# karknu/ouroboros-consensus

Hardware: AMD Instinct MI355X
Metric: Praos headers validated/sec (VRF+KES+OCert+leader) (higher is better)
Workload: dtype u32 (GF(2^255-19) radix-2^32 limbs; Fixed E34 bignum); 1 GPU; configs[4]: mainnet-shaped epoch replay, the first 432k blocks of a first-leader-wins Praos chain per GPU, 3000-pool stake distribution, single eta0, 1% corrupted; items_per_gpu=432000, items_total=432000, pools=3000, active_slot_coeff=1/20, signed_body=canonical HeaderBody CBOR, parallelism=shard-by-slot-range x1

## Files before the change

### ouroboros-consensus_amd/csrc/api_internal.hpp

```cpp
#pragma once
#include "praos_hip.h"
#include "launch.hpp"
#include "host_util.hpp"
#include "replay_internal.hpp"
#include "chunk_scan.hpp"
#include "sched.hpp"

static constexpr size_t NT = 256;
static constexpr size_t NIELS_BYTES = 3 * 32;
static constexpr size_t BTAB_N = 128;
static constexpr size_t BCOMB_TABLES = 32;
static constexpr size_t C16_TABLES = 16, C16_ENTRIES = 32768;
static constexpr size_t CACHED_BYTES = 4 * 32;
static constexpr size_t LT_ED_B = 8 * CACHED_BYTES, LT_VRF_B = 16 * CACHED_BYTES;
static constexpr size_t VRF_MID_BYTES = 28 * 16;
static constexpr uint32_t TP_SIGNED_STRIDE = 640;

#include <pthread.h>
#include <sched.h>

#include <algorithm>
#include <array>
#include <chrono>
#include <condition_variable>
#include <cstdlib>
#include <cstdio>
#include <cstring>
#include <functional>
#include <map>
// ... 385 lines not shown
```

### ouroboros-consensus_amd/csrc/k_selftest.hpp

```cpp
#pragma once
#include "kcommon.hpp"

#if PRAOS_ILP4
#define ST_LAUNCH(name) launch_selftest4_##name
#else
#define ST_LAUNCH(name) launch_selftest_##name
#endif

template <int BUILD>
__global__ void __launch_bounds__(64) k_selftest_fe_multi(int op, size_t n, const uint8_t* __restrict__ in,
                                                          uint8_t* __restrict__ out) {
  const size_t i = (size_t)blockIdx.x * blockDim.x + threadIdx.x;
  if (i >= n) return;
  fe a[4], b[4], r[4];
#pragma unroll
  for (int m = 0; m < 4; m++) {
    load_words(a[m].v, in + 256 * i + 64 * m, 8);
    load_words(b[m].v, in + 256 * i + 64 * m + 32, 8);
    fe_set(r[m], 0);
  }
  switch (op) {
    case 0: fe_mul2(r[0], a[0], b[0], r[1], a[1], b[1]); break;
    case 1: fe_sq2(r[0], a[0], r[1], a[1]); break;
    case 2: fe_mul3(r[0], a[0], b[0], r[1], a[1], b[1], r[2], a[2], b[2]); break;
// ... 178 lines not shown
    load_words(s1, sp + 32 * i, 8);
    load_words(s2, sq + 32 * i, 8);
    ge_p3 H, G;
    ge_frombytes(H, pk, false);
    load_words(pk, Qenc + 32 * i, 8);
    ge_frombytes(G, pk, false);
    fe_neg(G.X, G.X);
    fe_neg(G.T, G.T);
    ge_cached* vt = lane_tab(tabs, i, 16);
    build_cached_table(vt, H);
    build_cached_table(vt + 8, G);
    sc_recode16(w1, s1);
    sc_recode16(w2, s2);
    STRAUS<64, 64, 33, 0, false>(x, vt, w1, vt + 8, w2, nullptr, nullptr);
    ge_p1p1_to_p2(R, x);
  } else if constexpr (V == 3) {
    load_words(s1, sp + 32 * i, 8);
    load_words(s2, sb + 32 * i, 8);
    sc_recode16(w1, s1);
    sc_recode65536(w2, s2);
    straus_comb<16, false>(x, ktab + i * KT_STRIDE, w1, comb, w2);
    ge_p1p1_to_p2(R, x);
  } else if constexpr (V == 4) {
    load_words(s1, sp + 32 * i, 8);
    load_words(s2, sb + 32 * i, 8);
    sc_recode16(w1, s1);
    sc_recode65536(w2, s2);
    straus_comb<8, true>(x, ktab + i * KT_STRIDE, w1, comb, w2);
    ge_p1p1_to_p2(R, x);
  } else if constexpr (V == 6) {
// ... 2 lines not shown
    sc_recode65536(w2, s2);
    straus_pos(x, ktab + i * WT_STRIDE, s1, comb, w2);
    ge_p1p1_to_p2(R, x);
  } else {
    load_words(pk, Penc + 32 * i, 8);
    load_words(s1, sp + 32 * i, 8);
    ge_p3 P, S;
    ge_frombytes(P, pk, false);
    ge_scalarmult_var(S, s1, P);
    ge_p3_to_p2(R, S);
  }
  ge_tobytes(enc, R.X, R.Y, R.Z);
  store_words(out + 32 * i, enc, 8);
}

#if !PRAOS_ILP4
template <int BUILD>
__global__ void __launch_bounds__(64) k_selftest_int(int op, size_t n, const uint8_t* __restrict__ a,
                                                     const uint8_t* __restrict__ b, const uint8_t* __restrict__ c,
                                                     uint8_t* __restrict__ out) {
  const size_t i = (size_t)blockIdx.x * blockDim.x + threadIdx.x;
  if (i >= n) return;
  uint32_t x[8], y[8], z[8], r[8];
  load_words(x, a + 32 * i, 8);
#pragma unroll
  for (int k = 0; k < 8; k++) { y[k] = 0; z[k] = 0; r[k] = 0; }
  if (op == 1) {
    load_words(y, b + 32 * i, 8);
    load_words(z, c + 32 * i, 8);
  }
  if (op == 8) load_words(y, b + 32 * i, 8);
// ... 8 lines not shown
      uint32_t w[5];
      sc_recode64(w, x);
#pragma unroll
      for (int k = 0; k < 5; k++) r[k] = w[k];
    } break;
    case 7: fx_div_R(r, x); break;
    case 8: mp_div_small(r, x, y[0]); break;
    default: break;
  }
  store_words(out + 32 * i, r, 8);
}
#endif

void ST_LAUNCH(ge)(hipStream_t stream, int op, size_t n, const uint8_t* p, const uint8_t* q, uint8_t* out,
                   const ge_niels* gbtab) {
  hipLaunchKernelGGL(k_selftest_ge<PRAOS_ILP4>, dim3((unsigned)((n + 63) / 64)), dim3(64), 0, stream, op, n, p, q, out,
                     gbtab);
}
void ST_LAUNCH(msm)(hipStream_t stream, int variant, size_t n, const uint8_t* P, const uint8_t* Q, const uint8_t* sp,
                    const uint8_t* sq, const uint8_t* sb, const ge_niels* gbtab, const ge_niels* comb, ge_cached* tabs,
                    const ge_cached* ktab, uint8_t* out) {
  const dim3 grid((unsigned)((n + NT - 1) / NT)), block(NT);
#define ST_MSM(V)                                                                                                  \
  case V:                                                                                                          \
    hipLaunchKernelGGL((k_selftest_msm<PRAOS_ILP4, V>), grid, block, 0, stream, n, P, Q, sp, sq, sb, gbtab, comb, \
                       tabs, ktab, out);                                                                           \
    break
  switch (variant) {
    ST_MSM(0);
    ST_MSM(1);
    ST_MSM(2);
    ST_MSM(3);
    ST_MSM(4);
    ST_MSM(5);
    ST_MSM(6);
    default: break;
  }
#undef ST_MSM
}
#if !PRAOS_ILP4
void launch_selftest_fe_multi(hipStream_t stream, int op, size_t n, const uint8_t* in, uint8_t* out) {
  hipLaunchKernelGGL(k_selftest_fe_multi<0>, dim3((unsigned)((n + 63) / 64)), dim3(64), 0, stream, op, n, in, out);
}
void launch_selftest_fe(hipStream_t stream, int op, size_t n, const uint8_t* a, const uint8_t* b, uint8_t* r) {
  hipLaunchKernelGGL(k_selftest_fe<0>, dim3((unsigned)((n + 63) / 64)), dim3(64), 0, stream, op, n, a, b, r);
}
void launch_selftest_int(hipStream_t stream, int op, size_t n, const uint8_t* a, const uint8_t* b, const uint8_t* c,
                         uint8_t* out) {
  hipLaunchKernelGGL(k_selftest_int<0>, dim3((unsigned)((n + 63) / 64)), dim3(64), 0, stream, op, n, a, b, c, out);
}
#endif
```

### ouroboros-consensus_amd/csrc/k_vrf_stage.hip

```cpp
#include "k_vrf.hpp"

#ifndef LB_VRF_V
#define LB_VRF_V LB_VRF
#endif
#ifndef LB_VRF_F
#define LB_VRF_F LB_VRF
#endif
#ifndef LB_VRF_J
#define LB_VRF_J LB_VRF_F
#endif

__global__ void __launch_bounds__(NT, LB_VRF_V) k_vrf_v(size_t n, size_t i0, size_t i1, VrfIn a, uint4* __restrict__ mid) {
  const size_t i = i0 + (size_t)blockIdx.x * blockDim.x + threadIdx.x;
  if (i >= i1) return;
  if (a.wave_prio) __builtin_amdgcn_s_setprio(3);
  uint32_t pk[8], pr[20], alpha[8];
  load_words(pk, a.vrf_vk + 32 * i, 8);
  load_words(pr, a.vrf_proof + 80 * i, 20);
  header_alpha(alpha, a, i);
  vrf_v_core(mid, n, i, pk, pr, pr + 8, pr + 12, alpha, lane_tab(a.tabs, i, LT_VRF));
}

template <int CACHED>
__device__ __forceinline__ void vrf_fin_item(const VrfIn& a, size_t i, size_t stride, const uint4* __restrict__ mid,
// ... 76 lines not shown
}

__global__ void __launch_bounds__(NT, LB_VRF_J) k_vrf_fin_nc(size_t n, const uint32_t* __restrict__ list,
                                                           const uint32_t* __restrict__ count,
                                                           const ge_niels* __restrict__ gbtab, VrfIn a,
                                                           const uint4* __restrict__ mid) {
  const size_t items = list ? (size_t)*count : n;
  if ((size_t)blockIdx.x * NT >= items) return;
  __shared__ ge_niels sbtab[2 * BTAB_N];
  const ge_niels* btab = stage_btab<5>(gbtab, sbtab);
  const size_t t = (size_t)blockIdx.x * NT + threadIdx.x;
  if (t >= items) return;
  vrf_fin_item<false>(a, list ? list[t] : t, n, mid, btab, nullptr, nullptr);
}

__global__ void __launch_bounds__(NT, LB_VRF_F) k_vrf_u(size_t stride, const uint32_t* __restrict__ list,
                                                      const uint32_t* __restrict__ count,
                                                      const int32_t* __restrict__ item_entry,
                                                      const ge_cached* __restrict__ ktab,
                                                      const uint32_t* __restrict__ kinfo,
                                                      const ge_niels* __restrict__ comb,
                                                      const uint8_t* __restrict__ vrf_proof, uint4* __restrict__ mid,
                                                      int prio) {
  const size_t t = (size_t)blockIdx.x * blockDim.x + threadIdx.x;
  if (t >= (size_t)*count) return;
  wave_setprio(prio);
  const size_t i = list[t];
  const size_t e = (size_t)item_entry[i];
  uint32_t pr[20];
  load_words(pr, vrf_proof + 80 * i, 20);
  vrf_u_core<true>(mid, stride, i, nullptr, pr + 8, pr + 12, comb, nullptr, ktab + e * KT_STRIDE, kinfo + 9 * e);
// ... 297 lines not shown
```

### ouroboros-consensus_amd/csrc/kcommon.hpp

```cpp
#pragma once
#include "praos_core.hpp"
#include "leader.hpp"
#include "praos_hip.h"
#include "launch.hpp"

#define NT 256
#ifndef LB_ED
#define LB_ED 3
#endif
#ifndef LB_VRF
#define LB_VRF 3
#endif

#define LT_ED 8
#define LT_VRF 16
__device__ __forceinline__ ge_cached* lane_tab(ge_cached* __restrict__ arena, size_t i, int entries) {
  return arena + i * (size_t)entries;
}

__device__ __forceinline__ void load_words(uint32_t* w, const uint8_t* p, int nwords) {
  const uint4* q = (const uint4*)p;
  for (int i = 0; i < nwords / 4; i++) {
    const uint4 v = q[i];
    w[4 * i] = v.x; w[4 * i + 1] = v.y; w[4 * i + 2] = v.z; w[4 * i + 3] = v.w;
  }
}
__device__ __forceinline__ void store_words(uint8_t* p, const uint32_t* w, int nwords) {
  uint4* q = (uint4*)p;
  for (int i = 0; i < nwords / 4; i++) q[i] = make_uint4(w[4 * i], w[4 * i + 1], w[4 * i + 2], w[4 * i + 3]);
}
// ... 23 lines not shown
```

### ouroboros-consensus_amd/csrc/launch.hpp

```cpp
#pragma once
#include <hip/hip_runtime.h>
#include <cstddef>
#include <cstdint>
static inline unsigned lat_block(size_t n) { (void)n; return 256u; }
struct ge_niels;
struct ge_cached;
void launch_ocert(dim3 grid, dim3 block, hipStream_t stream, size_t n, const uint32_t* list, const uint32_t* count,
                  const ge_niels* gbtab, const uint8_t* cold_vk, const uint8_t* hot_vk, const uint64_t* ocert_n,
                  const uint64_t* ocert_c0, const uint8_t* sig, const uint64_t* slot, uint64_t slots_per_kes_period,
                  uint64_t max_kes_evo, uint16_t* bits, uint8_t* ok_out, ge_cached* tabs);
void launch_ocert_ck(dim3 grid, dim3 block, hipStream_t stream, const uint32_t* list, const uint32_t* count,
                     const int32_t* item_entry, const ge_cached* ktab, const uint32_t* kinfo, const ge_niels* gbtab,
                     const uint8_t* cold_vk, const uint8_t* hot_vk, const uint64_t* ocert_n, const uint64_t* ocert_c0,
                     const uint8_t* sig, const uint64_t* slot, uint64_t slots_per_kes_period, uint64_t max_kes_evo,
                     uint16_t* bits, uint8_t* ok_out, int prio = 0);
void launch_vrf(dim3 grid, dim3 block, hipStream_t stream, size_t n, const uint32_t* list, const uint32_t* count,
                const ge_niels* gbtab, const uint8_t* cold_vk, const uint8_t* vrf_vk, const uint8_t* vrf_out,
                const uint8_t* vrf_proof, const uint64_t* slot, const uint32_t* eta0, int eta0_neutral,
                const uint8_t* eta_idx, const uint32_t* pool_hash, const uint32_t* pool_vrf, const int32_t* pool_map,
                uint32_t npools, int check_output, const uint8_t* alpha_in, uint16_t* bits, int32_t* pool_idx,
                int32_t* pool_sorted_idx, uint8_t* beta_out, uint8_t* leader_out, uint8_t* nonce_out, uint8_t* ok_out,
                ge_cached* tabs);
void launch_vrf_ck(dim3 grid, dim3 block, hipStream_t stream, const uint32_t* list, const uint32_t* count,
                   const int32_t* item_entry, const ge_cached* ktab, const uint32_t* kinfo, const ge_niels* gbtab,
// ... 243 lines not shown
void launch_vrf_nonce(hipStream_t stream, size_t n, const uint8_t* vrf_out, int tpraos, uint8_t* nonce_out);
void launch_selftest_fe_multi(hipStream_t stream, int op, size_t n, const uint8_t* in, uint8_t* out);
void launch_selftest_fe(hipStream_t stream, int op, size_t n, const uint8_t* a, const uint8_t* b, uint8_t* r);
void launch_selftest_int(hipStream_t stream, int op, size_t n, const uint8_t* a, const uint8_t* b, const uint8_t* c,
                         uint8_t* out);
void launch_selftest_ge(hipStream_t stream, int op, size_t n, const uint8_t* p, const uint8_t* q, uint8_t* out,
                        const ge_niels* gbtab);
void launch_selftest4_ge(hipStream_t stream, int op, size_t n, const uint8_t* p, const uint8_t* q, uint8_t* out,
                         const ge_niels* gbtab);
void launch_selftest_msm(hipStream_t stream, int variant, size_t n, const uint8_t* P, const uint8_t* Q,
                         const uint8_t* sp, const uint8_t* sq, const uint8_t* sb, const ge_niels* gbtab,
                         const ge_niels* comb, ge_cached* tabs, const ge_cached* ktab, uint8_t* out);
void launch_selftest4_msm(hipStream_t stream, int variant, size_t n, const uint8_t* P, const uint8_t* Q,
                          const uint8_t* sp, const uint8_t* sq, const uint8_t* sb, const ge_niels* gbtab,
                          const ge_niels* comb, ge_cached* tabs, const ge_cached* ktab, uint8_t* out);
void launch_selftest_hash(hipStream_t stream, int kind, size_t n, const uint8_t* arena, const uint64_t* off,
                          const uint32_t* len, const uint8_t* aux, const uint64_t* parts, uint8_t* out);
void launch_wire_split(hipStream_t stream, size_t n, const uint8_t* arena, uint64_t arena_len, const uint64_t* off,
                       const uint32_t* len, uint32_t n_eras, uint8_t* status, uint8_t* era, uint8_t* kind,
                       uint32_t* hint, uint64_t* ioff, uint32_t* ilen, uint8_t* hash);
void launch_hdr_dedup(hipStream_t stream, size_t n, const uint8_t* status, const uint8_t* era, const uint8_t* hash,
                      uint32_t era_mask, uint32_t mask, uint32_t* slot_item, uint32_t* slot_min, uint32_t* item_slot,
                      uint32_t* item_rep, uint32_t* blk, uint32_t* total, const uint64_t* ioff, const uint32_t* ilen,
                      uint32_t rows_cap, uint64_t* row_off, uint32_t* row_len, uint32_t* rep_row, uint32_t* item_row);
void launch_hdr_row_kind(hipStream_t stream, size_t n, const uint32_t* item_slot, const uint32_t* item_rep,
                         const uint32_t* rep_row, const uint8_t* kind, uint32_t rows_cap, uint8_t* row_is_ebb);
```

### ouroboros-consensus_amd/csrc/praos_core.hpp

```cpp
#pragma once
#include "hash.hpp"
#include "scalarmult.hpp"
#include "sc25519.hpp"

FE_INLINE uint32_t fsh16(uint32_t hi, uint32_t lo) { return __builtin_amdgcn_alignbit(hi, lo, 16); }

template <int NW, int NBYTES>
FE_INLINE void sha512_regs(uint32_t out[16], const uint32_t S[NW]) {
  constexpr int NBLK = (NBYTES + 17 + 127) / 128;
  uint64_t H[8];
  sha512_init(H);
#pragma unroll
  for (int b = 0; b < NBLK; b++) {
    uint64_t W[16];
#pragma unroll
    for (int w = 0; w < 16; w++) {
      const int i0 = 32 * b + 2 * w, i1 = i0 + 1;
      const uint32_t lo = i0 < NW ? S[i0] : 0u;
      const uint32_t hi = i1 < NW ? S[i1] : 0u;
      W[w] = bswap64(((uint64_t)hi << 32) | lo);
    }
    if (b == NBLK - 1) W[15] = (uint64_t)NBYTES * 8u;
    sha512_block(H, W);
  }
// ... 379 lines not shown
  mid_put(mid, stride, i, plane + 4, Z.v);
}
FE_INLINE void mid_get_xyz(fe& X, fe& Y, fe& Z, const uint4* __restrict__ mid, size_t stride, size_t i, int plane) {
  mid_get(X.v, mid, stride, i, plane);
  mid_get(Y.v, mid, stride, i, plane + 2);
  mid_get(Z.v, mid, stride, i, plane + 4);
}

FE_INLINE void vrf_key_canonical(uint32_t ys[8], const uint32_t pk[8]) {
  fe y;
  fe_frombytes32(y, pk);
  fe_tobytes32(ys, y);
  ys[7] |= pk[7] & 0x80000000u;
}

FE_INLINE void vrf_v_core(uint4* __restrict__ mid, size_t stride, size_t i, const uint32_t pk[8],
                          const uint32_t gamma[8], const uint32_t c4[4], const uint32_t s8[8],
                          const uint32_t alpha[8], ge_cached* __restrict__ vt) {
  {
    uint32_t ys[8];
    vrf_key_canonical(ys, pk);
    ge_p3 H;
    vrf_hash_to_curve(H, ys, alpha);
    mid_put_xyz(mid, stride, i, VRF_MID_H, H.X, H.Y, H.Z);
    build_cached_table(vt, H);
  }
  {
    ge_p3 G;
    const bool gamma_ok = ge_frombytes(G, gamma, false);
    uint32_t gs[8];
    ge_enc_affine(gs, G);
    mid_put(mid, stride, i, VRF_MID_GS, gs);
    mid[(size_t)VRF_MID_FLAGS * stride + i] = make_uint4(gamma_ok ? 1u : 0u, 0u, 0u, 0u);
    fe_neg(G.X, G.X);
    fe_neg(G.T, G.T);
    ge_p3 G8;
    build_cached_table(vt + 8, G, &G8);
    fe_neg(G8.X, G8.X);
    mid_put_xyz(mid, stride, i, VRF_MID_G8, G8.X, G8.Y, G8.Z);
  }
  uint32_t sx[16], s[8], c[8], sw[8], cw[8];
#pragma unroll
  for (int k = 0; k < 16; k++) sx[k] = k < 8 ? s8[k] : 0u;
  sc_reduce512(s, sx);
#pragma unroll
  for (int k = 0; k < 8; k++) c[k] = k < 4 ? c4[k] : 0u;
  sc_recode16(sw, s);
  sc_recode16(cw, c);
  ge_p1p1 x;
  STRAUS<64, 64, 33, 0, false>(x, vt, sw, vt + 8, cw, nullptr, nullptr);
  ge_p2 V;
  ge_p1p1_to_p2(V, x);
  mid_put_xyz(mid, stride, i, VRF_MID_V, V.X, V.Y, V.Z);
}

template <int CACHED>
FE_INLINE bool vrf_fin_core(uint32_t beta[16], bool& gamma_ok, const uint4* __restrict__ mid, size_t stride,
                            size_t i, const uint32_t pk[8], const uint32_t c4[4], const uint32_t s8[8],
                            const ge_niels* __restrict__ btab, ge_cached* __restrict__ vt,
                            const ge_cached* __restrict__ ktab, const uint32_t* __restrict__ kinfo) {
  bool ok;
  uint32_t sx[16], s[8], c[8], cw[8], sw[8];
#pragma unroll
  for (int k = 0; k < 16; k++) sx[k] = k < 8 ? s8[k] : 0u;
  sc_reduce512(s, sx);
// ... 229 lines not shown
```

### ouroboros-consensus_amd/csrc/praos_debug.hip

```cpp
#include "api_internal.hpp"

using namespace praos_impl;

namespace {
struct Scratch {
  praos_ctx* c;
  std::vector<void*> ptrs;
  bool ok = true;
  explicit Scratch(praos_ctx* cc) : c(cc) {}
  ~Scratch() { for (void* p : ptrs) (void)hipFree(p); }
  template <typename T>
  T* up(const T* src, size_t bytes) {
    void* d = nullptr;
    if (hipMalloc(&d, bytes ? bytes : 16) != hipSuccess) { ok = false; return nullptr; }
    ptrs.push_back(d);
    if (src && bytes && hipMemcpy(d, src, bytes, hipMemcpyHostToDevice) != hipSuccess) ok = false;
    return (T*)d;
  }
  template <typename T>
  T* zeros(size_t bytes) {
    T* d = up<T>(nullptr, bytes);
    if (d && hipMemsetAsync(d, 0, bytes ? bytes : 16, c->stream) != hipSuccess) ok = false;
    return d;
  }
// ... 495 lines not shown
  HIPCHK(c, hipGetLastError());
  HIPCHK(c, hipStreamSynchronize(c->stream));
  HIPCHK(c, hipMemcpy(out, dout, 128 * n, hipMemcpyDeviceToHost));
  return PRAOS_OK;
}

static bool scalars_below(const uint8_t* s, size_t n, int bits) {
  for (size_t i = 0; i < n; i++)
    for (int k = bits / 8; k < 32; k++)
      if (k == bits / 8 ? (s[32 * i + k] >> (bits % 8)) != 0 : s[32 * i + k] != 0) return false;
  return true;
}

int praos_debug_msm(praos_ctx* c, int variant, int build, size_t n, const uint8_t* P, const uint8_t* Q,
                    const uint8_t* sp, const uint8_t* sq, const uint8_t* sb, uint8_t* out) {
  if (!c || !out || variant < 0 || variant > 6 || build < 0 || build > 1 || !P || !sp) return PRAOS_E_ARG;
  const bool use_q = variant == 2, use_b = variant != 2 && variant != 5;
  const bool wide = variant == 6, cached = variant == 3 || variant == 4 || wide;
  if (wide && n > 4096) return PRAOS_E_ARG;
  if ((use_q && (!Q || !sq)) || (use_b && !sb)) return PRAOS_E_ARG;
  if (n == 0) return PRAOS_OK;
  if (n > (1u << 20)) return PRAOS_E_ARG;
  if (!scalars_below(sp, n, (variant == 1 || variant == 4 || wide) ? 128 : 253)) return PRAOS_E_ARG;
  if (use_q && !scalars_below(sq, n, 128)) return PRAOS_E_ARG;
  if (use_b && !scalars_below(sb, n, 253)) return PRAOS_E_ARG;
  HIPCHK(c, hipSetDevice(c->device));
  if (cached) {
    const int rc = ensure_bcomb16(c);
    if (rc != PRAOS_OK) return rc;
  }
  Scratch s(c);
  auto dP = s.up(P, 32 * n);
// ... 12 lines not shown
    auto drep = s.up(rep.data(), 4 * n);
    auto dcnt = s.up(cnt, sizeof cnt);
    auto kinfo = s.zeros<uint32_t>(9 * 4 * n);
    ktab = s.zeros<ge_cached>(KT_BYTES * n);
    KeyWide w;
    if (wide) {
      w.min_uses = 1;
      w.cap = (uint32_t)n;
      w.wide_ent = drep;
      w.wcnt = dcnt;
      w.wtab = s.zeros<ge_cached>(WT_BYTES * n);
      w.wbase = s.zeros<ge_cached>(WT_BYTES / 32 * n);
    }
    if (!s.ok) return PRAOS_E_OOM;
    launch_key_precompute(variant == 3 ? 0 : 1, c->stream, dcnt, (uint32_t)n, drep, dP, ktab, kinfo, 0, nullptr,
                          (uint32_t)n, build, w);
    if (wide) ktab = w.wtab;
  } else {
    tabs = s.zeros<ge_cached>(LT_VRF_B * n);
  }
  if (!s.ok) return PRAOS_E_OOM;
  if (build) launch_selftest4_msm(c->stream, variant, n, dP, dQ, dsp, dsq, dsb, c->btab, c->bcomb16, tabs, ktab, dout);
  else launch_selftest_msm(c->stream, variant, n, dP, dQ, dsp, dsq, dsb, c->btab, c->bcomb16, tabs, ktab, dout);
  HIPCHK(c, hipGetLastError());
  HIPCHK(c, hipStreamSynchronize(c->stream));
  HIPCHK(c, hipMemcpy(out, dout, 32 * n, hipMemcpyDeviceToHost));
  return PRAOS_OK;
}

int praos_debug_hash_bytes(praos_ctx* c, int kind, size_t n, const uint8_t* arena, size_t arena_len,
                           const uint64_t* off, const uint32_t* len, const uint8_t* aux, const uint64_t* parts,
                           size_t n_parts, uint8_t* out) {
  if (!c || kind < 0 || kind > 4 || (!arena && arena_len) || n > (1u << 24) || n_parts > (1u << 26))
    return PRAOS_E_ARG;
  if (n == 0) return PRAOS_OK;
  const bool stream = kind >= 3;
  const size_t items = kind == 2 ? 4 * n : n, out_len = kind == 3 ? 64 : 32;
// ... 82 lines not shown
```

### ouroboros-consensus_amd/csrc/scalarmult.hpp

```cpp
#pragma once
#include "ge25519.hpp"

#define BTAB_N 128
#define BTAB_WORDS (BTAB_N * 24)

FE_INLINE void sc_recode16(uint32_t w[8], const uint32_t s[8]) {
  uint32_t c = 0;
#pragma unroll
  for (int i = 0; i < 8; i++) w[i] = addc(s[i], 0x88888888u, c, &c);
}
FE_INLINE void sc_recode256(uint32_t w[8], const uint32_t s[8]) {
  uint32_t c = 0;
#pragma unroll
  for (int i = 0; i < 8; i++) w[i] = addc(s[i], 0x80808080u, c, &c);
}

template <int NW, int SH>
FE_INLINE void shl_small(uint32_t w[NW]) {
#pragma unroll
  for (int i = NW - 1; i > 0; i--) w[i] = __builtin_amdgcn_alignbit(w[i], w[i - 1], 32 - SH);
  w[0] <<= SH;
}
template <int NW, int BITS>
FE_INLINE void shl_const(uint32_t w[NW]) {
  constexpr int WS = BITS / 32, B = BITS % 32;
  if constexpr (WS > 0) {
#pragma unroll
    for (int i = NW - 1; i >= 0; i--) w[i] = i >= WS ? w[i - WS] : 0u;
  }
  if constexpr (B > 0) shl_small<NW, B>(w);
}

FE_INLINE void build_cached_table(ge_cached* __restrict__ tab, const ge_p3& P, ge_p3* last = nullptr) {
  ge_p3 acc, P2;
  ge_p1p1 t;
  ge_p3_to_cached(tab[0], P);
  ge_p3_dbl_to_p3(P2, P);
  ge_p3_to_cached(tab[1], P2);
  acc = P2;
#pragma clang loop unroll(disable)
  for (int k = 2; k < 8; k++) {
    ge_add(t, acc, tab[0]);
    ge_p1p1_to_p3(acc, t);
    ge_p3_to_cached(tab[k], acc);
  }
  if (last) *last = acc;
}

FE_INLINE void cached_fix(ge_cached& c, bool zero, bool neg) {
#pragma unroll
  for (int i = 0; i < 8; i++) {
    c.YpX.v[i] = zero ? (i == 0 ? 1u : 0u) : c.YpX.v[i];
    c.YmX.v[i] = zero ? (i == 0 ? 1u : 0u) : c.YmX.v[i];
    c.Z.v[i] = zero ? (i == 0 ? 1u : 0u) : c.Z.v[i];
    c.T2d.v[i] = zero ? 0u : c.T2d.v[i];
  }
  ge_cached_cneg(c, neg);
}
FE_INLINE void niels_fix(ge_niels& c, bool zero, bool neg) {
#pragma unroll
  for (int i = 0; i < 8; i++) {
    c.ypx.v[i] = zero ? (i == 0 ? 1u : 0u) : c.ypx.v[i];
    c.ymx.v[i] = zero ? (i == 0 ? 1u : 0u) : c.ymx.v[i];
    c.xy2d.v[i] = zero ? 0u : c.xy2d.v[i];
  }
  ge_niels_cneg(c, neg);
}
FE_INLINE void select_cached(ge_cached& c, const ge_cached tab[8], int d) {
  const int a = d < 0 ? -d : d;
  c = tab[a == 0 ? 0 : a - 1];
  cached_fix(c, a == 0, d < 0);
}
FE_INLINE void select_niels(ge_niels& c, const ge_niels* __restrict__ tab, int d) {
  const int a = d < 0 ? -d : d;
  c = tab[a == 0 ? 0 : a - 1];
  niels_fix(c, a == 0, d < 0);
}

FE_INLINE void dbl4_p1p1(ge_p1p1& x, const ge_p2& acc) {
  ge_p2 q = acc;
  ge_p2_dbl(x, q); ge_p1p1_to_p2(q, x);
  ge_p2_dbl(x, q); ge_p1p1_to_p2(q, x);
  ge_p2_dbl(x, q); ge_p1p1_to_p2(q, x);
  ge_p2_dbl(x, q);
}

FE_INLINE void ge_p1p1_identity(ge_p1p1& x) { fe_set(x.X, 0); fe_set(x.Y, 1); fe_set(x.Z, 1); fe_set(x.T, 1); }

template <int NWIN, int NP, int NQ, int NB, bool TWO_B>
FE_INLINE void straus(ge_p1p1& out, const ge_cached* tp, uint32_t pw[8], const ge_cached* tq, uint32_t qw[8],
                      const ge_niels* __restrict__ btab, uint32_t fw[8]) {
  static_assert(NWIN >= 1 && NWIN <= 64 && NP <= NWIN && NQ <= NWIN, "window counts");
  static_assert(NB == 0 || (NB == 32 && !TWO_B) || (NB == 16 && TWO_B), "fixed-base layout");
  static_assert(NB == 0 || 2 * (NB - 1) <= NWIN - 1, "fixed-base bytes beyond the chain");
  static_assert(NB == 0 || NWIN - 1 <= 2 * NB, "chain starts above the top fixed-base byte");
  if constexpr (NP > 0) shl_const<8, 4 * (64 - NWIN)>(pw);
  if constexpr (NQ > 0) shl_const<8, 4 * (64 - NWIN)>(qw);
  ge_p2 acc;
  ge_p1p1 x;
  ge_p3 a3;
#pragma clang loop unroll(disable)
  for (int j = NWIN - 1; j >= 0; j--) {
    if (j == NWIN - 1) ge_p1p1_identity(x);
    else dbl4_p1p1(x, acc);
    if constexpr (NP > 0) {
      if (j < NP) {
        ge_cached c;
        select_cached(c, tp, (int)(pw[7] >> 28) - 8);
        ge_p1p1_to_p3(a3, x);
        ge_add(x, a3, c);
      }
      shl_small<8, 4>(pw);
    }
    if constexpr (NQ > 0) {
      if (j < NQ) {
        ge_cached c;
        select_cached(c, tq, (int)(qw[7] >> 28) - 8);
        ge_p1p1_to_p3(a3, x);
        ge_add(x, a3, c);
      }
      shl_small<8, 4>(qw);
    }
    if constexpr (NB > 0) {
      if ((j & 1) == 0 && (j >> 1) < NB) {
        ge_niels nb;
        if constexpr (TWO_B) {
          select_niels(nb, btab, (int)(fw[3] >> 24) - 128);
          ge_p1p1_to_p3(a3, x);
          ge_madd(x, a3, nb);
          select_niels(nb, btab + BTAB_N, (int)(fw[7] >> 24) - 128);
          ge_p1p1_to_p3(a3, x);
          ge_madd(x, a3, nb);
          shl_small<4, 8>(fw);
          shl_small<4, 8>(fw + 4);
        } else {
          select_niels(nb, btab, (int)(fw[7] >> 24) - 128);
          ge_p1p1_to_p3(a3, x);
          ge_madd(x, a3, nb);
          shl_small<8, 8>(fw);
        }
      }
    }
    if (j > 0) ge_p1p1_to_p2(acc, x);
  }
  out = x;
}

#ifndef PRAOS_ROLLED
#define PRAOS_ROLLED 1
#endif

FE_INLINE void dbl4_rolled(ge_p1p1& x) {
#pragma clang loop unroll(disable)
  for (int k = 0; k < 4; k++) {
    ge_p2 q;
    ge_p1p1_to_p2(q, x);
    ge_p2_dbl(x, q);
  }
}
FE_INLINE void add_cached_sel(ge_p1p1& x, const ge_cached* __restrict__ tab, int d) {
  const int a = d < 0 ? -d : d;
  ge_cached c = tab[a == 0 ? 0 : a - 1];
  ge_p3 a3;
  ge_p1p1_to_p3(a3, x);
  cached_fix(c, a == 0, d < 0);
  ge_add(x, a3, c);
}
FE_INLINE void add_niels_sel(ge_p1p1& x, const ge_niels* __restrict__ tab, int d) {
  const int a = d < 0 ? -d : d;
  ge_niels c = tab[a == 0 ? 0 : a - 1];
  ge_p3 a3;
  ge_p1p1_to_p3(a3, x);
  niels_fix(c, a == 0, d < 0);
  ge_madd(x, a3, c);
}

template <int NWIN, int NP, int NQ, int NB, bool TWO_B>
FE_INLINE void straus_rolled(ge_p1p1& out, const ge_cached* tp, uint32_t pw[8], const ge_cached* tq,
                             uint32_t qw[8], const ge_niels* __restrict__ btab, uint32_t fw[8]) {
  static_assert(NWIN >= 1 && NWIN <= 64 && NP <= NWIN && NQ <= NP, "window counts (terms ordered NQ <= NP)");
  static_assert(NB == 0 || (NB == 32 && !TWO_B) || (NB == 16 && TWO_B), "fixed-base layout");
  static_assert(NB == 0 || 2 * (NB - 1) <= NWIN - 1, "fixed-base bytes beyond the chain");
  static_assert(NB == 0 || NWIN - 1 <= 2 * NB, "chain starts above the top fixed-base byte");
  if constexpr (NP > 0) shl_const<8, 4 * (64 - NWIN)>(pw);
  if constexpr (NQ > 0) shl_const<8, 4 * (64 - NWIN)>(qw);
  ge_p1p1 x;
  ge_p1p1_identity(x);
#pragma clang loop unroll(disable)
  for (int j = NWIN - 1; j >= 0; j--) {
    if (j != NWIN - 1) dbl4_rolled(x);
    if constexpr (NP > 0) {
      const int nt = (NQ > 0 && j < NQ) ? 2 : (j < NP ? 1 : 0);
#pragma clang loop unroll(disable)
      for (int t = 0; t < nt; t++) {
        uint32_t top = pw[7];
        if constexpr (NQ > 0) top = t == 0 ? pw[7] : qw[7];
        add_cached_sel(x, (NQ > 0 && t != 0) ? tq : tp, (int)(top >> 28) - 8);
      }
      shl_small<8, 4>(pw);
      if constexpr (NQ > 0) shl_small<8, 4>(qw);
    }
    if constexpr (NB > 0) {
      if ((j & 1) == 0 && (j >> 1) < NB) {
        constexpr int NT2 = TWO_B ? 2 : 1;
#pragma clang loop unroll(disable)
        for (int t = 0; t < NT2; t++) {
          const uint32_t top = TWO_B ? (t == 0 ? fw[3] : fw[7]) : fw[7];
          add_niels_sel(x, btab + BTAB_N * t, (int)(top >> 24) - 128);
        }
        if constexpr (TWO_B) {
          shl_small<4, 8>(fw);
          shl_small<4, 8>(fw + 4);
        } else {
          shl_small<8, 8>(fw);
        }
      }
    }
  }
  out = x;
}

FE_INLINE void ge_scalarmult_base(ge_p3& R, const uint32_t s[8], const ge_niels* __restrict__ btab) {
  uint32_t fw[8];
  sc_recode256(fw, s);
  ge_p1p1 x;
  straus<31, 0, 0, 16, true>(x, nullptr, nullptr, nullptr, nullptr, btab, fw);
  ge_p1p1_to_p3(R, x);
}

FE_INLINE void ge_scalarmult_var(ge_p3& R, const uint32_t s[8], const ge_p3& P) {
  ge_cached tab[8];
  build_cached_table(tab, P);
  uint32_t pw[8];
  sc_recode16(pw, s);
  ge_p1p1 x;
  straus<64, 64, 0, 0, false>(x, tab, pw, nullptr, nullptr, nullptr, nullptr);
// ... 13 lines not shown
}

template <int N>
FE_INLINE uint32_t word_sel(const uint32_t w[8], int k) {
  uint32_t r = w[0];
#pragma unroll
  for (int i = 1; i < N; i++) r = k == i ? w[i] : r;
  return r;
}

template <int NPC, bool P_TOP>
FE_INLINE void straus_comb(ge_p1p1& out, const ge_cached* __restrict__ ktab, const uint32_t pw[8],
                           const ge_niels* __restrict__ comb, const uint32_t fw[8]) {
  static_assert(NPC >= 1 && NPC + (P_TOP ? 1 : 0) <= KT_CHUNKS, "chunk count");
  ge_p1p1 x;
  ge_p1p1_identity(x);
#pragma clang loop unroll(disable)
  for (int m = 3; m >= 0; m--) {
    if (m != 3) dbl4_rolled(x);
    const int nt = NPC + ((P_TOP && m == 0) ? 1 : 0);
#pragma clang loop unroll(disable)
    for (int k = 0; k < nt; k++) {
      const uint32_t w = word_sel<(NPC + 2) / 2>(pw, k >> 1);
      add_cached_sel(x, ktab + 8 * k, (int)((w >> (16 * (k & 1) + 4 * m)) & 15u) - 8);
    }
  }
#pragma clang loop unroll(disable)
  for (int j = 0; j < C16_T; j++) {
    const uint32_t w = word_sel<8>(fw, j >> 1);
    add_niels_sel(x, comb + (size_t)C16_N * j, (int)((w >> (16 * (j & 1))) & 0xffffu) - 32768);
  }
  out = x;
}

#define WT_POS 22
#define WT_N 32
#define WT_STRIDE (WT_POS * WT_N)

FE_INLINE void sc_recode64(uint32_t w[5], const uint32_t c[4]) {
  uint32_t cy = 0;
  w[0] = addc(c[0], 0x20820820u, cy, &cy);
  w[1] = addc(c[1], 0x08208208u, cy, &cy);
  w[2] = addc(c[2], 0x82082082u, cy, &cy);
  w[3] = addc(c[3], 0x20820820u, cy, &cy);
  w[4] = 8u + cy;
}

FE_INLINE void straus_pos(ge_p1p1& out, const ge_cached* __restrict__ wtab, const uint32_t p[4],
                          const ge_niels* __restrict__ comb, const uint32_t fw[8]) {
  uint32_t w[5];
  sc_recode64(w, p);
  ge_p1p1 x;
  ge_p1p1_identity(x);
#pragma clang loop unroll(disable)
  for (int k = 0; k < WT_POS; k++) {
    add_cached_sel(x, wtab + WT_N * k, (int)(w[0] & 63u) - 32);
#pragma unroll
    for (int i = 0; i < 4; i++) w[i] = __builtin_amdgcn_alignbit(w[i + 1], w[i], 6);
    w[4] >>= 6;
  }
#pragma clang loop unroll(disable)
  for (int j = 0; j < C16_T; j++) {
    const uint32_t d = word_sel<8>(fw, j >> 1);
    add_niels_sel(x, comb + (size_t)C16_N * j, (int)((d >> (16 * (j & 1))) & 0xffffu) - 32768);
  }
  out = x;
}

FE_INLINE void key_pos_bases(ge_cached* __restrict__ wbase, const ge_p3& Qk, int k) {
  ge_p3 Q = Qk;
#pragma clang loop unroll(disable)
// ... 78 lines not shown
```

Measured before the change: 44.00 million headers/s.

## Use radix-32 signed window for VRF s*H, start chains from first table entry

The VRF verification double-scalar multiply now recodes the full scalar s into 51 signed 5-bit digits over a 16-entry table of H, instead of 64 nibbles over 8 entries. This cuts the number of point additions for the H term, while the 128-bit challenge keeps its radix-16 schedule inside one shared doubling loop. Straus, comb and positional chains now start by loading the first selected table entry directly rather than adding it to the identity, which saves one full addition per chain. The G table is built with a cheaper addition that assumes Z=1. The per-lane table arena grows from 16 to 24 entries, which adds memory traffic and register pressure. A separate launch-bounds macro for k_vrf_u is also added, plus a reference selftest build that keeps the old paths for checking.

New measurement: 44.36 million headers/s, median of 6. Within noise of the previous version (+0.8%).

```diff
diff --git a/ouroboros-consensus_amd/csrc/api_internal.hpp b/ouroboros-consensus_amd/csrc/api_internal.hpp
--- a/ouroboros-consensus_amd/csrc/api_internal.hpp
+++ b/ouroboros-consensus_amd/csrc/api_internal.hpp
@@ -12,7 +12,7 @@
 static constexpr size_t BCOMB_TABLES = 32;
 static constexpr size_t C16_TABLES = 16, C16_ENTRIES = 32768;
 static constexpr size_t CACHED_BYTES = 4 * 32;
-static constexpr size_t LT_ED_B = 8 * CACHED_BYTES, LT_VRF_B = 16 * CACHED_BYTES;
+static constexpr size_t LT_ED_B = 8 * CACHED_BYTES, LT_VRF_B = 24 * CACHED_BYTES;
 static constexpr size_t VRF_MID_BYTES = 28 * 16;
 static constexpr uint32_t TP_SIGNED_STRIDE = 640;
 
diff --git a/ouroboros-consensus_amd/csrc/k_selftest.hpp b/ouroboros-consensus_amd/csrc/k_selftest.hpp
--- a/ouroboros-consensus_amd/csrc/k_selftest.hpp
+++ b/ouroboros-consensus_amd/csrc/k_selftest.hpp
@@ -1,10 +1,15 @@
 #pragma once
 #include "kcommon.hpp"
 
-#if PRAOS_ILP4
+#if PRAOS_ST_REF
+#define ST_LAUNCH(name) launch_selftest_ref_##name
+#define ST_BUILD 2
+#elif PRAOS_ILP4
 #define ST_LAUNCH(name) launch_selftest4_##name
+#define ST_BUILD 1
 #else
 #define ST_LAUNCH(name) launch_selftest_##name
+#define ST_BUILD 0
 #endif
 
 template <int BUILD>
@@ -216,6 +221,28 @@
     sc_recode16(w2, s2);
     STRAUS<64, 64, 33, 0, false>(x, vt, w1, vt + 8, w2, nullptr, nullptr);
     ge_p1p1_to_p2(R, x);
+  } else if constexpr (V == 7) {
+    load_words(pk, Penc + 32 * i, 8);
+    load_words(s1, sp + 32 * i, 8);
+    load_words(s2, sq + 32 * i, 8);
+    ge_p3 H, G;
+    ge_frombytes(H, pk, false);
+    load_words(pk, Qenc + 32 * i, 8);
+    ge_frombytes(G, pk, false);
+    fe_neg(G.X, G.X);
+    fe_neg(G.T, G.T);
+    ge_cached* vt = lane_tab(tabs, i, LT_VRF);
+    build_cached_table<VRF_VT_H>(vt, H);
+    build_cached_table<8, true>(vt + VRF_VT_H, G);
+    sc_recode16(w2, s2);
+#if PRAOS_V32
+    sc_recode32(w1, s1);
+    straus_v32(x, vt, w1, vt + VRF_VT_H, w2);
+#else
+    sc_recode16(w1, s1);
+    STRAUS<64, 64, 33, 0, false>(x, vt, w1, vt + VRF_VT_H, w2, nullptr, nullptr);
+#endif
+    ge_p1p1_to_p2(R, x);
   } else if constexpr (V == 3) {
     load_words(s1, sp + 32 * i, 8);
     load_words(s2, sb + 32 * i, 8);
@@ -248,7 +275,7 @@
   store_words(out + 32 * i, enc, 8);
 }
 
-#if !PRAOS_ILP4
+#if ST_BUILD == 0
 template <int BUILD>
 __global__ void __launch_bounds__(64) k_selftest_int(int op, size_t n, const uint8_t* __restrict__ a,
                                                      const uint8_t* __restrict__ b, const uint8_t* __restrict__ c,
@@ -287,7 +314,7 @@
 
 void ST_LAUNCH(ge)(hipStream_t stream, int op, size_t n, const uint8_t* p, const uint8_t* q, uint8_t* out,
                    const ge_niels* gbtab) {
-  hipLaunchKernelGGL(k_selftest_ge<PRAOS_ILP4>, dim3((unsigned)((n + 63) / 64)), dim3(64), 0, stream, op, n, p, q, out,
+  hipLaunchKernelGGL(k_selftest_ge<ST_BUILD>, dim3((unsigned)((n + 63) / 64)), dim3(64), 0, stream, op, n, p, q, out,
                      gbtab);
 }
 void ST_LAUNCH(msm)(hipStream_t stream, int variant, size_t n, const uint8_t* P, const uint8_t* Q, const uint8_t* sp,
@@ -296,7 +323,7 @@
   const dim3 grid((unsigned)((n + NT - 1) / NT)), block(NT);
 #define ST_MSM(V)                                                                                                  \
   case V:                                                                                                          \
-    hipLaunchKernelGGL((k_selftest_msm<PRAOS_ILP4, V>), grid, block, 0, stream, n, P, Q, sp, sq, sb, gbtab, comb, \
+    hipLaunchKernelGGL((k_selftest_msm<ST_BUILD, V>), grid, block, 0, stream, n, P, Q, sp, sq, sb, gbtab, comb, \
                        tabs, ktab, out);                                                                           \
     break
   switch (variant) {
@@ -307,11 +334,12 @@
     ST_MSM(4);
     ST_MSM(5);
     ST_MSM(6);
+    ST_MSM(7);
     default: break;
   }
 #undef ST_MSM
 }
-#if !PRAOS_ILP4
+#if ST_BUILD == 0
 void launch_selftest_fe_multi(hipStream_t stream, int op, size_t n, const uint8_t* in, uint8_t* out) {
   hipLaunchKernelGGL(k_selftest_fe_multi<0>, dim3((unsigned)((n + 63) / 64)), dim3(64), 0, stream, op, n, in, out);
 }
diff --git a/ouroboros-consensus_amd/csrc/k_selftest_ref.hip b/ouroboros-consensus_amd/csrc/k_selftest_ref.hip
--- /dev/null
+++ b/ouroboros-consensus_amd/csrc/k_selftest_ref.hip
@@ -0,0 +1,8 @@
+#undef PRAOS_CHAIN_START
+#undef PRAOS_V32
+#undef PRAOS_TAB_Z1
+#define PRAOS_CHAIN_START 0
+#define PRAOS_V32 0
+#define PRAOS_TAB_Z1 0
+#define PRAOS_ST_REF 1
+#include "k_selftest.hpp"
diff --git a/ouroboros-consensus_amd/csrc/k_vrf_stage.hip b/ouroboros-consensus_amd/csrc/k_vrf_stage.hip
--- a/ouroboros-consensus_amd/csrc/k_vrf_stage.hip
+++ b/ouroboros-consensus_amd/csrc/k_vrf_stage.hip
@@ -8,6 +8,9 @@
 #endif
 #ifndef LB_VRF_J
 #define LB_VRF_J LB_VRF_F
+#endif
+#ifndef LB_VRF_U
+#define LB_VRF_U 4
 #endif
 
 __global__ void __launch_bounds__(NT, LB_VRF_V) k_vrf_v(size_t n, size_t i0, size_t i1, VrfIn a, uint4* __restrict__ mid) {
@@ -114,7 +117,7 @@
   vrf_fin_item<false>(a, list ? list[t] : t, n, mid, btab, nullptr, nullptr);
 }
 
-__global__ void __launch_bounds__(NT, LB_VRF_F) k_vrf_u(size_t stride, const uint32_t* __restrict__ list,
+__global__ void __launch_bounds__(NT, LB_VRF_U) k_vrf_u(size_t stride, const uint32_t* __restrict__ list,
                                                       const uint32_t* __restrict__ count,
                                                       const int32_t* __restrict__ item_entry,
                                                       const ge_cached* __restrict__ ktab,
diff --git a/ouroboros-consensus_amd/csrc/kcommon.hpp b/ouroboros-consensus_amd/csrc/kcommon.hpp
--- a/ouroboros-consensus_amd/csrc/kcommon.hpp
+++ b/ouroboros-consensus_amd/csrc/kcommon.hpp
@@ -13,7 +13,8 @@
 #endif
 
 #define LT_ED 8
-#define LT_VRF 16
+#define LT_VRF 24
+static_assert(LT_VRF == VRF_VT, "stage V's table region");
 __device__ __forceinline__ ge_cached* lane_tab(ge_cached* __restrict__ arena, size_t i, int entries) {
   return arena + i * (size_t)entries;
 }
diff --git a/ouroboros-consensus_amd/csrc/launch.hpp b/ouroboros-consensus_amd/csrc/launch.hpp
--- a/ouroboros-consensus_amd/csrc/launch.hpp
+++ b/ouroboros-consensus_amd/csrc/launch.hpp
@@ -281,6 +281,9 @@
 void launch_selftest4_msm(hipStream_t stream, int variant, size_t n, const uint8_t* P, const uint8_t* Q,
                           const uint8_t* sp, const uint8_t* sq, const uint8_t* sb, const ge_niels* gbtab,
                           const ge_niels* comb, ge_cached* tabs, const ge_cached* ktab, uint8_t* out);
+void launch_selftest_ref_msm(hipStream_t stream, int variant, size_t n, const uint8_t* P, const uint8_t* Q,
+                             const uint8_t* sp, const uint8_t* sq, const uint8_t* sb, const ge_niels* gbtab,
+                             const ge_niels* comb, ge_cached* tabs, const ge_cached* ktab, uint8_t* out);
 void launch_selftest_hash(hipStream_t stream, int kind, size_t n, const uint8_t* arena, const uint64_t* off,
                           const uint32_t* len, const uint8_t* aux, const uint64_t* parts, uint8_t* out);
 void launch_wire_split(hipStream_t stream, size_t n, const uint8_t* arena, uint64_t arena_len, const uint64_t* off,
diff --git a/ouroboros-consensus_amd/csrc/praos_core.hpp b/ouroboros-consensus_amd/csrc/praos_core.hpp
--- a/ouroboros-consensus_amd/csrc/praos_core.hpp
+++ b/ouroboros-consensus_amd/csrc/praos_core.hpp
@@ -417,6 +417,11 @@
   ys[7] |= pk[7] & 0x80000000u;
 }
 
+#ifndef PRAOS_V32
+#define PRAOS_V32 1
+#endif
+#define VRF_VT_H (PRAOS_V32 ? V32_TAB : 8)
+#define VRF_VT (V32_TAB + 8)
 FE_INLINE void vrf_v_core(uint4* __restrict__ mid, size_t stride, size_t i, const uint32_t pk[8],
                           const uint32_t gamma[8], const uint32_t c4[4], const uint32_t s8[8],
                           const uint32_t alpha[8], ge_cached* __restrict__ vt) {
@@ -426,7 +431,7 @@
     ge_p3 H;
     vrf_hash_to_curve(H, ys, alpha);
     mid_put_xyz(mid, stride, i, VRF_MID_H, H.X, H.Y, H.Z);
-    build_cached_table(vt, H);
+    build_cached_table<VRF_VT_H>(vt, H);
   }
   {
     ge_p3 G;
@@ -438,7 +443,7 @@
     fe_neg(G.X, G.X);
     fe_neg(G.T, G.T);
     ge_p3 G8;
-    build_cached_table(vt + 8, G, &G8);
+    build_cached_table<8, true>(vt + VRF_VT_H, G, &G8);
     fe_neg(G8.X, G8.X);
     mid_put_xyz(mid, stride, i, VRF_MID_G8, G8.X, G8.Y, G8.Z);
   }
@@ -448,10 +453,15 @@
   sc_reduce512(s, sx);
 #pragma unroll
   for (int k = 0; k < 8; k++) c[k] = k < 4 ? c4[k] : 0u;
-  sc_recode16(sw, s);
   sc_recode16(cw, c);
   ge_p1p1 x;
-  STRAUS<64, 64, 33, 0, false>(x, vt, sw, vt + 8, cw, nullptr, nullptr);
+#if PRAOS_V32
+  sc_recode32(sw, s);
+  straus_v32(x, vt, sw, vt + VRF_VT_H, cw);
+#else
+  sc_recode16(sw, s);
+  STRAUS<64, 64, 33, 0, false>(x, vt, sw, vt + VRF_VT_H, cw, nullptr, nullptr);
+#endif
   ge_p2 V;
   ge_p1p1_to_p2(V, x);
   mid_put_xyz(mid, stride, i, VRF_MID_V, V.X, V.Y, V.Z);
diff --git a/ouroboros-consensus_amd/csrc/praos_debug.hip b/ouroboros-consensus_amd/csrc/praos_debug.hip
--- a/ouroboros-consensus_amd/csrc/praos_debug.hip
+++ b/ouroboros-consensus_amd/csrc/praos_debug.hip
@@ -533,8 +533,8 @@
 
 int praos_debug_msm(praos_ctx* c, int variant, int build, size_t n, const uint8_t* P, const uint8_t* Q,
                     const uint8_t* sp, const uint8_t* sq, const uint8_t* sb, uint8_t* out) {
-  if (!c || !out || variant < 0 || variant > 6 || build < 0 || build > 1 || !P || !sp) return PRAOS_E_ARG;
-  const bool use_q = variant == 2, use_b = variant != 2 && variant != 5;
+  if (!c || !out || variant < 0 || variant > 7 || build < 0 || build > 2 || !P || !sp) return PRAOS_E_ARG;
+  const bool use_q = variant == 2 || variant == 7, use_b = !use_q && variant != 5;
   const bool wide = variant == 6, cached = variant == 3 || variant == 4 || wide;
   if (wide && n > 4096) return PRAOS_E_ARG;
   if ((use_q && (!Q || !sq)) || (use_b && !sb)) return PRAOS_E_ARG;
@@ -577,13 +577,16 @@
     }
     if (!s.ok) return PRAOS_E_OOM;
     launch_key_precompute(variant == 3 ? 0 : 1, c->stream, dcnt, (uint32_t)n, drep, dP, ktab, kinfo, 0, nullptr,
-                          (uint32_t)n, build, w);
+                          (uint32_t)n, build == 1, w);
     if (wide) ktab = w.wtab;
   } else {
     tabs = s.zeros<ge_cached>(LT_VRF_B * n);
   }
   if (!s.ok) return PRAOS_E_OOM;
-  if (build) launch_selftest4_msm(c->stream, variant, n, dP, dQ, dsp, dsq, dsb, c->btab, c->bcomb16, tabs, ktab, dout);
+  if (build == 2)
+    launch_selftest_ref_msm(c->stream, variant, n, dP, dQ, dsp, dsq, dsb, c->btab, c->bcomb16, tabs, ktab, dout);
+  else if (build)
+    launch_selftest4_msm(c->stream, variant, n, dP, dQ, dsp, dsq, dsb, c->btab, c->bcomb16, tabs, ktab, dout);
   else launch_selftest_msm(c->stream, variant, n, dP, dQ, dsp, dsq, dsb, c->btab, c->bcomb16, tabs, ktab, dout);
   HIPCHK(c, hipGetLastError());
   HIPCHK(c, hipStreamSynchronize(c->stream));
diff --git a/ouroboros-consensus_amd/csrc/scalarmult.hpp b/ouroboros-consensus_amd/csrc/scalarmult.hpp
--- a/ouroboros-consensus_amd/csrc/scalarmult.hpp
+++ b/ouroboros-consensus_amd/csrc/scalarmult.hpp
@@ -13,6 +13,21 @@
   uint32_t c = 0;
 #pragma unroll
   for (int i = 0; i < 8; i++) w[i] = addc(s[i], 0x80808080u, c, &c);
+}
+
+constexpr uint32_t sc_rc32_word(int i) {
+  uint32_t v = 0;
+  for (int k = 0; k < 51; k++)
+    if ((5 * k + 4) / 32 == i) v |= 1u << ((5 * k + 4) % 32);
+  return v;
+}
+static_assert(sc_rc32_word(0) == 0x21084210u && sc_rc32_word(7) == 0x42108421u, "radix-32 recoding constant");
+FE_INLINE void sc_recode32(uint32_t w[8], const uint32_t s[8]) {
+  constexpr uint32_t K[8] = {sc_rc32_word(0), sc_rc32_word(1), sc_rc32_word(2), sc_rc32_word(3),
+                             sc_rc32_word(4), sc_rc32_word(5), sc_rc32_word(6), sc_rc32_word(7)};
+  uint32_t c = 0;
+#pragma unroll
+  for (int i = 0; i < 8; i++) w[i] = addc(s[i], K[i], c, &c);
 }
 
 template <int NW, int SH>
@@ -31,7 +46,30 @@
   if constexpr (B > 0) shl_small<NW, B>(w);
 }
 
+#ifndef PRAOS_TAB_Z1
+#define PRAOS_TAB_Z1 1
+#endif
+
+FE_INLINE void ge_add_z1(ge_p1p1& r, const ge_p3& p, const ge_cached& q) {
+  fe t0;
+  fe_add(r.X, p.Y, p.X);
+  fe_sub(r.Y, p.Y, p.X);
+#if PRAOS_ILP4
+  fe_mul3(r.Z, r.X, q.YpX, r.Y, r.Y, q.YmX, r.T, q.T2d, p.T);
+#else
+  fe_mul2(r.Z, r.X, q.YpX, r.Y, r.Y, q.YmX);
+  fe_mul(r.T, q.T2d, p.T);
+#endif
+  fe_add(t0, p.Z, p.Z);
+  fe_sub(r.X, r.Z, r.Y);
+  fe_add(r.Y, r.Z, r.Y);
+  fe_add(r.Z, t0, r.T);
+  fe_sub(r.T, t0, r.T);
+}
+
+template <int N = 8, bool Z1 = false>
 FE_INLINE void build_cached_table(ge_cached* __restrict__ tab, const ge_p3& P, ge_p3* last = nullptr) {
+  static_assert(N >= 2, "entry count");
   ge_p3 acc, P2;
   ge_p1p1 t;
   ge_p3_to_cached(tab[0], P);
@@ -39,8 +77,9 @@
   ge_p3_to_cached(tab[1], P2);
   acc = P2;
 #pragma clang loop unroll(disable)
-  for (int k = 2; k < 8; k++) {
-    ge_add(t, acc, tab[0]);
+  for (int k = 2; k < N; k++) {
+    if constexpr (Z1 && PRAOS_TAB_Z1) ge_add_z1(t, acc, tab[0]);
+    else ge_add(t, acc, tab[0]);
     ge_p1p1_to_p3(acc, t);
     ge_p3_to_cached(tab[k], acc);
   }
@@ -66,7 +105,7 @@
   }
   ge_niels_cneg(c, neg);
 }
-FE_INLINE void select_cached(ge_cached& c, const ge_cached tab[8], int d) {
+FE_INLINE void select_cached(ge_cached& c, const ge_cached* tab, int d) {
   const int a = d < 0 ? -d : d;
   c = tab[a == 0 ? 0 : a - 1];
   cached_fix(c, a == 0, d < 0);
@@ -76,6 +115,23 @@
   c = tab[a == 0 ? 0 : a - 1];
   niels_fix(c, a == 0, d < 0);
 }
+
+#ifndef PRAOS_CHAIN_START
+#define PRAOS_CHAIN_START 1
+#endif
+FE_INLINE void start_cached(ge_p1p1& x, const ge_cached& c) {
+  fe_sub(x.X, c.YpX, c.YmX);
+  fe_add(x.Y, c.YpX, c.YmX);
+  fe_add(x.Z, c.Z, c.Z);
+  x.T = x.Z;
+}
+FE_INLINE void start_niels(ge_p1p1& x, const ge_niels& c) {
+  fe_sub(x.X, c.ypx, c.ymx);
+  fe_add(x.Y, c.ypx, c.ymx);
+  fe_set(x.Z, 2);
+  fe_set(x.T, 2);
+}
+FE_INLINE void start_to_p2(ge_p2& q, const ge_p1p1& x) { q.X = x.X; q.Y = x.Y; q.Z = x.Z; }
 
 FE_INLINE void dbl4_p1p1(ge_p1p1& x, const ge_p2& acc) {
   ge_p2 q = acc;
@@ -103,12 +159,19 @@
   for (int j = NWIN - 1; j >= 0; j--) {
     if (j == NWIN - 1) ge_p1p1_identity(x);
     else dbl4_p1p1(x, acc);
+    bool fresh = PRAOS_CHAIN_START && j == NWIN - 1, sform = false;
     if constexpr (NP > 0) {
       if (j < NP) {
         ge_cached c;
         select_cached(c, tp, (int)(pw[7] >> 28) - 8);
-        ge_p1p1_to_p3(a3, x);
-        ge_add(x, a3, c);
+        if (fresh) {
+          start_cached(x, c);
+        } else {
+          ge_p1p1_to_p3(a3, x);
+          ge_add(x, a3, c);
+        }
+        sform = fresh;
+        fresh = false;
       }
       shl_small<8, 4>(pw);
     }
@@ -116,8 +179,14 @@
       if (j < NQ) {
         ge_cached c;
         select_cached(c, tq, (int)(qw[7] >> 28) - 8);
-        ge_p1p1_to_p3(a3, x);
-        ge_add(x, a3, c);
+        if (fresh) {
+          start_cached(x, c);
+        } else {
+          ge_p1p1_to_p3(a3, x);
+          ge_add(x, a3, c);
+        }
+        sform = fresh;
+        fresh = false;
       }
       shl_small<8, 4>(qw);
     }
@@ -126,22 +195,36 @@
         ge_niels nb;
         if constexpr (TWO_B) {
           select_niels(nb, btab, (int)(fw[3] >> 24) - 128);
-          ge_p1p1_to_p3(a3, x);
-          ge_madd(x, a3, nb);
+          if (fresh) {
+            start_niels(x, nb);
+          } else {
+            ge_p1p1_to_p3(a3, x);
+            ge_madd(x, a3, nb);
+          }
           select_niels(nb, btab + BTAB_N, (int)(fw[7] >> 24) - 128);
           ge_p1p1_to_p3(a3, x);
           ge_madd(x, a3, nb);
+          sform = false;
           shl_small<4, 8>(fw);
           shl_small<4, 8>(fw + 4);
         } else {
           select_niels(nb, btab, (int)(fw[7] >> 24) - 128);
-          ge_p1p1_to_p3(a3, x);
-          ge_madd(x, a3, nb);
+          if (fresh) {
+            start_niels(x, nb);
+          } else {
+            ge_p1p1_to_p3(a3, x);
+            ge_madd(x, a3, nb);
+          }
+          sform = fresh;
           shl_small<8, 8>(fw);
         }
+        fresh = false;
       }
     }
-    if (j > 0) ge_p1p1_to_p2(acc, x);
+    if (j > 0) {
+      if (sform) start_to_p2(acc, x);
+      else ge_p1p1_to_p2(acc, x);
+    }
   }
   out = x;
 }
@@ -150,11 +233,12 @@
 #define PRAOS_ROLLED 1
 #endif
 
-FE_INLINE void dbl4_rolled(ge_p1p1& x) {
+FE_INLINE void dbl4_rolled(ge_p1p1& x, bool sform = false) {
 #pragma clang loop unroll(disable)
   for (int k = 0; k < 4; k++) {
     ge_p2 q;
-    ge_p1p1_to_p2(q, x);
+    if (sform && k == 0) start_to_p2(q, x);
+    else ge_p1p1_to_p2(q, x);
     ge_p2_dbl(x, q);
   }
 }
@@ -165,6 +249,12 @@
   ge_p1p1_to_p3(a3, x);
   cached_fix(c, a == 0, d < 0);
   ge_add(x, a3, c);
+}
+FE_INLINE void start_cached_sel(ge_p1p1& x, const ge_cached* __restrict__ tab, int d) {
+  const int a = d < 0 ? -d : d;
+  ge_cached c = tab[a == 0 ? 0 : a - 1];
+  cached_fix(c, a == 0, d < 0);
+  start_cached(x, c);
 }
 FE_INLINE void add_niels_sel(ge_p1p1& x, const ge_niels* __restrict__ tab, int d) {
   const int a = d < 0 ? -d : d;
@@ -184,15 +274,18 @@
   static_assert(NB == 0 || NWIN - 1 <= 2 * NB, "chain starts above the top fixed-base byte");
   if constexpr (NP > 0) shl_const<8, 4 * (64 - NWIN)>(pw);
   if constexpr (NQ > 0) shl_const<8, 4 * (64 - NWIN)>(qw);
-  ge_p1p1 x;
-  ge_p1p1_identity(x);
+  constexpr bool START = PRAOS_CHAIN_START && NP == NWIN;
+  constexpr bool TOP_ALONE = NQ < NWIN && !(NB > 0 && ((NWIN - 1) & 1) == 0 && ((NWIN - 1) >> 1) < NB);
+  ge_p1p1 x;
+  if constexpr (START) start_cached_sel(x, tp, (int)(pw[7] >> 28) - 8);
+  else ge_p1p1_identity(x);
 #pragma clang loop unroll(disable)
   for (int j = NWIN - 1; j >= 0; j--) {
-    if (j != NWIN - 1) dbl4_rolled(x);
+    if (j != NWIN - 1) dbl4_rolled(x, START && TOP_ALONE && j == NWIN - 2);
     if constexpr (NP > 0) {
       const int nt = (NQ > 0 && j < NQ) ? 2 : (j < NP ? 1 : 0);
 #pragma clang loop unroll(disable)
-      for (int t = 0; t < nt; t++) {
+      for (int t = (START && j == NWIN - 1) ? 1 : 0; t < nt; t++) {
         uint32_t top = pw[7];
         if constexpr (NQ > 0) top = t == 0 ? pw[7] : qw[7];
         add_cached_sel(x, (NQ > 0 && t != 0) ? tq : tp, (int)(top >> 28) - 8);
@@ -220,6 +313,40 @@
   out = x;
 }
 
+#define V32_DIGITS 51
+#define V32_TAB 16
+FE_INLINE void straus_v32(ge_p1p1& out, const ge_cached* tp, uint32_t pw[8], const ge_cached* tq, uint32_t qw[8]) {
+  constexpr int TOP = 5 * (V32_DIGITS - 1);
+  static_assert(TOP + 5 == 255 && TOP > 4 * 32, "51 digits of 5 bits; the top one above Q's nibbles");
+  shl_small<8, 1>(pw);
+  shl_const<8, 4 * (64 - 33)>(qw);
+  ge_p1p1 x;
+#if PRAOS_CHAIN_START
+  start_cached_sel(x, tp, (int)(pw[7] >> 27) - 16);
+#else
+  ge_p1p1_identity(x);
+#endif
+#pragma clang loop unroll(disable)
+  for (int b = TOP; b >= 0; b--) {
+    if (b != TOP) {
+      ge_p2 q;
+      if (PRAOS_CHAIN_START && b == TOP - 1) start_to_p2(q, x);
+      else ge_p1p1_to_p2(q, x);
+      ge_p2_dbl(x, q);
+    }
+    const bool hp = b % 5 == 0, hq = (b & 3) == 0 && b < 4 * 33;
+    const int nt = (hp ? 1 : 0) + (hq ? 1 : 0);
+#pragma clang loop unroll(disable)
+    for (int t = (PRAOS_CHAIN_START && b == TOP) ? 1 : 0; t < nt; t++) {
+      const bool isp = hp && t == 0;
+      add_cached_sel(x, isp ? tp : tq, isp ? (int)(pw[7] >> 27) - 16 : (int)(qw[7] >> 28) - 8);
+    }
+    if (hp) shl_small<8, 5>(pw);
+    if (hq) shl_small<8, 4>(qw);
+  }
+  out = x;
+}
+
 FE_INLINE void ge_scalarmult_base(ge_p3& R, const uint32_t s[8], const ge_niels* __restrict__ btab) {
   uint32_t fw[8];
   sc_recode256(fw, s);
@@ -263,13 +390,17 @@
                            const ge_niels* __restrict__ comb, const uint32_t fw[8]) {
   static_assert(NPC >= 1 && NPC + (P_TOP ? 1 : 0) <= KT_CHUNKS, "chunk count");
   ge_p1p1 x;
+#if PRAOS_CHAIN_START
+  start_cached_sel(x, ktab, (int)((pw[0] >> 12) & 15u) - 8);
+#else
   ge_p1p1_identity(x);
+#endif
 #pragma clang loop unroll(disable)
   for (int m = 3; m >= 0; m--) {
     if (m != 3) dbl4_rolled(x);
     const int nt = NPC + ((P_TOP && m == 0) ? 1 : 0);
 #pragma clang loop unroll(disable)
-    for (int k = 0; k < nt; k++) {
+    for (int k = (PRAOS_CHAIN_START && m == 3) ? 1 : 0; k < nt; k++) {
       const uint32_t w = word_sel<(NPC + 2) / 2>(pw, k >> 1);
       add_cached_sel(x, ktab + 8 * k, (int)((w >> (16 * (k & 1) + 4 * m)) & 15u) - 8);
     }
@@ -300,10 +431,14 @@
   uint32_t w[5];
   sc_recode64(w, p);
   ge_p1p1 x;
+#if PRAOS_CHAIN_START
+  start_cached_sel(x, wtab, (int)(w[0] & 63u) - 32);
+#else
   ge_p1p1_identity(x);
+#endif
 #pragma clang loop unroll(disable)
   for (int k = 0; k < WT_POS; k++) {
-    add_cached_sel(x, wtab + WT_N * k, (int)(w[0] & 63u) - 32);
+    if (!PRAOS_CHAIN_START || k != 0) add_cached_sel(x, wtab + WT_N * k, (int)(w[0] & 63u) - 32);
 #pragma unroll
     for (int i = 0; i < 4; i++) w[i] = __builtin_amdgcn_alignbit(w[i + 1], w[i], 6);
     w[4] >>= 6;
```
